# feixue94/pram

Hardware: AMD Instinct MI355X
Metric: query images/sec (640x480, 2048 kpts, 7Scenes nc113) (higher is better)
Workload: dtype f32 results via split-fp16 MFMA (f16 x3 products, f32 accumulate); 1 GPU; 7Scenes full hot path: SFD2 extract+sample -> SegNetViT nc113 (15 layers) -> GML match + 20 Sinkhorn iters, 2048 query kpts vs a 2048-kpt reference set; stages=erm; precision=x3, batches_in_flight_per_gpu=3, hipgraph_replay=False, attention_chunk_keys=4096, frame=640x480, keypoints=2048, parallelism=query-sharded x1, one all-gather of result records, matches_last_step=14291, matches_correct_last_step=14288, gather_order_verified=True

## Files before the change

### include/pram_hip.h

```cpp
#ifndef PRAM_HIP_H
#define PRAM_HIP_H

#include <stddef.h>
#include <stdint.h>

#ifdef __cplusplus
extern "C" {
#endif

#define PRAM_OK 0
#define PRAM_E_ARG (-1)
#define PRAM_E_LAUNCH (-2)
#define PRAM_E_UNSUPPORTED (-3)

int pram_hip_version(void);
const char* pram_last_error(void);

#define PRAM_STATUS_X3_RANGE 1u
int pram_set_status_word(unsigned int* device_word);
float pram_x3_set_act_scale(float scale);
int pram_read_status_word(unsigned int* host_out, int reset, void* stream);


#define PRAM_LIN_ROTARY 1
// ... 182 lines not shown
int pram_score_map_f32(const float* logits, float* score, int batch, int hc, int wc, void* stream);

size_t pram_simple_nms_workspace_bytes(int batch, int h, int w);
int pram_simple_nms_f32(const float* score, float* nms, int batch, int h, int w, int radius,
                        void* workspace, void* stream);

size_t pram_select_keypoints_workspace_bytes(int batch, int h, int w, int max_keypoints);

int pram_select_keypoints_f32(const float* nms, int batch, int h, int w, float conf_th,
                              int min_keypoints, int border, int max_keypoints, int fallback_ref,
                              float* kpts, float* scores, int* counts, void* workspace, void* stream);

int pram_sample_nhwc_f32(const float* fmap, int batch, int fh, int fw, int c, const float* kpts,
                         const int* lens, int n_max, int s, int l2norm, float* out, void* stream);

int pram_l2norm_rows_f32(float* x, int rows, int cols, void* stream);

int pram_score_lookup_f32(const float* score_map, long long map_stride, int h, int w, const float* kpts,
                          const int* lens, int batch, int n_max, float* out, void* stream);


int pram_resize_bilinear_f32(const float* in, float* out, int planes, int h, int w, int oh, int ow,
                             void* stream);

int pram_seg_epilogue_f32(const float* logits, const int* lens, int batch, int n_max, int n_class,
                          float bg_threshold, float* seg_scores, int* seg_ids, int* non_bg_mask,
                          int* n_non_bg, void* stream);

int pram_row_sort_desc_f32(const float* x, int ld, int rows, int cols, float* vals, long long* idx,
                           void* stream);
// ... 92 lines not shown
```

### pram_amd/_lib.py

```python
from __future__ import annotations

import ctypes as C
from pathlib import Path

import os as _os
_LIB_PATH = Path(_os.environ["PRAM_HIP_LIB"]) if _os.environ.get("PRAM_HIP_LIB") else Path(__file__).resolve().parent / "csrc" / "libpram_hip.so"
_lib = None

P = C.c_void_p
I = C.c_int
F = C.c_float
LL = C.c_longlong
SZ = C.c_size_t

_SIGS = {
    "pram_hip_version": (I, []),
    "pram_last_error": (C.c_char_p, []),
    "pram_set_status_word": (I, [P]),
    "pram_read_status_word": (I, [P, I, P]),
    "pram_x3_set_act_scale": (F, [F]),
    "pram_linear_f32": (I, [P, I, I, P, I, I, P, P, P, I, P, I, I, I, F, I, P, P, I, P]),
    "pram_linear_f16_f32": (I, [P, I, I, P, I, I, P, P, P, I, P, I, I, I, F, I, P, P, I, P]),
    "pram_linear_f16_ragged_f32": (I, [P, I, I, P, I, I, P, P, P, I, P, I, I, I, F, I, P, P, I, P, I, P]),
    "pram_linear_f16_h16": (I, [P, I, I, P, I, I, P, P, P, I, P, I, P, I, I, I, F, I, P, P, I, P]),
# ... 42 lines not shown
    "pram_adagml_scores4_f32": (I, [P, P, P, LL, P]),
    "pram_adagml_prune_ld_f32": (I, [P, I, F, I, P, P, P, P, P, P, P, P, P, P, P, P, P, I, I, I, P]),
    "pram_adagml_scatter_f32": (I, [P, P, P, P, P, I, I, I, P, P, P]),
    "pram_conv2d_nhwc_f32": (I, [P, I, I, I, I, P, P, P, P, P, P, I, I, I, I, P]),
    "pram_conv2d_nhwc_f16_f32": (I, [P, I, I, I, I, P, P, P, P, P, P, I, I, I, I, P]),
    "pram_conv3x3_grouped_nhwc_f32": (I, [P, I, I, I, I, P, P, P, P, I, I, P]),
    "pram_image_to_nhwc4_f32": (I, [P, P, I, I, I, P]),
    "pram_nhwc_to_nchw_f32": (I, [P, P, I, I, I, I, P]),
    "pram_score_map_f32": (I, [P, P, I, I, I, P]),
    "pram_simple_nms_workspace_bytes": (SZ, [I, I, I]),
    "pram_simple_nms_f32": (I, [P, P, I, I, I, I, P, P]),
    "pram_select_keypoints_workspace_bytes": (SZ, [I, I, I, I]),
    "pram_select_keypoints_f32": (I, [P, I, I, I, F, I, I, I, I, P, P, P, P, P]),
    "pram_sample_nhwc_f32": (I, [P, I, I, I, I, P, P, I, I, I, P, P]),
    "pram_l2norm_rows_f32": (I, [P, I, I, P]),
    "pram_resize_bilinear_f32": (I, [P, P, I, I, I, I, I, P]),
    "pram_seg_epilogue_f32": (I, [P, P, I, I, I, F, P, P, P, P, P]),
    "pram_row_sort_desc_f32": (I, [P, I, I, I, P, P, P]),
    "pram_row_top2_f32": (I, [P, I, LL, P, P, I, I, I, I, P, P, P, P]),
    "pram_proj_dist_top2_f32": (I, [P, I, P, P, I, I, F, P, P, P, P]),
    "pram_proj_dist_top2_f64uv": (I, [P, I, P, P, I, I, I, C.c_double, P, P, P, P]),
    "pram_project_points_f64": (I, [P, P, P, I, C.c_double, C.c_double, P, P, P, P, P, P]),
    "pram_seg_vote": (I, [P, P, I, I, I, P, P, P, P, P, P, P]),
    "pram_pack_record_f32": (I, [P, P, P, P, P, I, I, I, P, P]),
    "pram_fill_u32": (I, [P, C.c_uint, SZ, P]),
    "pram_stage_frames_u8": (I, [P, P, P, I, I, I, P]),
    "pram_score_lookup_f32": (I, [P, LL, I, I, P, P, I, I, P, P]),
    "pram_cand_mask_ranks": (I, [P, P, I, I, I, P]),
    "pram_cand_plan": (I, [P, P, P, P, P, I, I, I, I, P, P, P, I, I, P, P, P, P, I, I, C.c_double, I, P, P]),
    "pram_cand_gather": (I, [P, P, P, P, P, P, I, P, P, P, P, I, F, F, F, P, P, P, P, P, P, I, I, P]),
# ... 44 lines not shown
```

### pram_amd/csrc/conv.hip

```cpp
#include <stdlib.h>
#include "gemm_core.h"
#include "gemm_core_f16.h"
#include "gemm_core_x3.h"
#include "gemm_core_x3w.h"
#include "launch.h"

namespace {

struct ConvArgs {
    const float* in; const float* w; const float* bias; const float* scale; const float* shift;
    const float* residual; float* out;
    int batch, h, wd, cin, cout, ks, stride, relu;
    int ho, wo, m, k;
    int tiles_m, tiles_n;
    unsigned int* status;
    _Float16* out_hi; _Float16* out_lo;
    float act_scale = gemmx3::ACT_SCALE;
};

template <int MI, int WN>
__device__ __forceinline__ void conv_epilogue(const ConvArgs& p, f32x16 (&acc)[MI][2], int row0, int col0, int BM, int BN) {
    using gemm::acc_row;
    const int tid = threadIdx.x;
    const int nlast = p.cout - 1;
    const int lane = tid & 63, wave = tid >> 6;
    const int wm = wave / WN, wn = wave % WN;
    const int r = lane & 31, h = lane >> 5;
    const int mlast = p.m - 1;
    const int rbase = row0 + wm * 32 * MI;
    const bool full = (row0 + BM <= p.m) && (col0 + BN <= p.cout);
#pragma unroll
    for (int ni = 0; ni < 2; ++ni) {
        const int col = col0 + wn * 64 + ni * 32 + r;
// ... 254 lines not shown
        const bool in = (unsigned)iy < (unsigned)p.h && (unsigned)ix < (unsigned)p.wd;
        const unsigned off = in ? (unsigned)(roff[pp] + tap) : 0u;
        return *reinterpret_cast<const float4*>(base[pp] + off);
    };
    auto oka = [&](int pp, int kt) -> bool {
        const int iy = iy0[pp] + cky, ix = ix0[pp] + ckx;
        return ok[pp] && (unsigned)iy < (unsigned)p.h && (unsigned)ix < (unsigned)p.wd;
    };
    auto lb = [&](int pp, int kt) -> uint4 { return *reinterpret_cast<const uint4*>(brow16[pp] + koff); };
    auto okb = [&](int pp, int kt) -> bool { return (col0 + brow + 32 * pp) < p.cout; };
    f32x16 acc[MI][2];
    mainloop<MI, WN>(smem, adv, la, oka, lb, okb, p.k / BK, acc);
    conv_epilogue<MI, WN>(p, acc, row0, col0, BM, BN);
}

template <int MI, int WN, bool L2N = false>
__global__ __launch_bounds__(gemmx3::NT, 2) void conv_x3_kernel(ConvArgs p, const _Float16* __restrict__ wh,
                                                                 const _Float16* __restrict__ wl, float inv) {
    using namespace gemmx3;
    using C = Cfg<MI, WN>;
    constexpr int BM = C::BM, BN = C::BN;
    __shared__ Smem<MI, WN> smem;
    const int nblk = p.tiles_m * p.tiles_n;
    const int id = xcd_remap(blockIdx.x, nblk);
    const int tn = id % p.tiles_n, tm = id / p.tiles_n;
    const int tid = threadIdx.x;
    const int arow = tid >> 3, akq = tid & 7, brow = tid >> 2, bsl = tid & 3;
    const int row0 = tm * BM, col0 = tn * BN;
    const int pad = p.ks >> 1;
    int iy0[C::PA], ix0[C::PA], roff[C::PA];
    const float* base[C::PA];
    bool ok[C::PA];
#pragma unroll
    for (int pp = 0; pp < C::PA; ++pp) {
        const int row = row0 + arow + 32 * pp;
        ok[pp] = row < p.m;
        const int rr = ok[pp] ? row : 0;
        const int ox = rr % p.wo;
        const int t = rr / p.wo;
        const int oy = t % p.ho;
        const int b = t / p.ho;
        iy0[pp] = oy * p.stride - pad;
        ix0[pp] = ox * p.stride - pad;
// ... 25 lines not shown
    auto okb = [&](int pp, int kt) -> bool { return (col0 + brow + 64 * pp) < p.cout; };
    f32x16 acc[MI][2];
    float amax = 0.f;
    mainloop<MI, WN>(smem, adv, la, oka, lb, okb, p.k / BK, p.act_scale, acc, amax);
    x3_range_flag(p.status, amax);
#pragma unroll
    for (int mi = 0; mi < MI; ++mi)
#pragma unroll
        for (int ni = 0; ni < 2; ++ni)
#pragma unroll
            for (int e = 0; e < 16; ++e) acc[mi][ni][e] *= inv;
    if constexpr (L2N) conv_epilogue_l2norm<MI, WN>(p, acc, row0, col0, BM, reinterpret_cast<float*>(&smem));
    else conv_epilogue<MI, WN>(p, acc, row0, col0, BM, BN);
}

template <int MI, int WM, int WN, bool PLANES = false>
__global__ __launch_bounds__(64 * WM * WN, 2) void conv_x3w_kernel(ConvArgs p, const _Float16* __restrict__ wh,
                                                                    const _Float16* __restrict__ wl, float inv) {
    using namespace gemmx3w;
    using C = Cfg<MI, WM, WN>;
    constexpr int BM = C::BM, BN = C::BN;
    extern __shared__ __attribute__((aligned(16))) unsigned char smem_raw[];
    Smem<MI, WM, WN>& smem = *reinterpret_cast<Smem<MI, WM, WN>*>(smem_raw);
    const int nblk = p.tiles_m * p.tiles_n;
    const int id = xcd_remap(blockIdx.x, nblk);
    const int tn = id % p.tiles_n, tm = id / p.tiles_n;
    const int tid = threadIdx.x;
    const int arow = tid >> 3, akq = tid & 7, qrow = tid >> 2, qsl = tid & 3;
    const int row0 = tm * BM, col0 = tn * BN;
    const int pad = p.ks >> 1;
    int iy0[C::PA], ix0[C::PA], roff[C::PA];
    const float* base[C::PA];
    bool ok[C::PA];
#pragma unroll
    for (int pp = 0; pp < C::PA; ++pp) {
        const int row = row0 + arow + C::RA * pp;
        ok[pp] = row < p.m;
        const int rr = ok[pp] ? row : 0;
        const int ox = rr % p.wo;
        const int t = rr / p.wo;
        const int oy = t % p.ho;
        const int b = t / p.ho;
        iy0[pp] = oy * p.stride - pad;
        ix0[pp] = ox * p.stride - pad;
        base[pp] = p.in + (size_t)b * p.h * p.wd * p.cin;
        roff[pp] = (iy0[pp] * p.wd + ix0[pp]) * p.cin + akq * 4;
    }
    const int nlast = p.cout - 1;
    int cky = 0, ckx = 0, cci = 0, koff = 0, tap = 0;
    auto adv = [&](int kt) {
        if (kt == 0) { cky = ckx = cci = koff = tap = 0; return; }
        if (++ckx == p.ks) { ckx = 0; if (++cky == p.ks) { cky = 0; cci += BK; } }
        koff = (cky * p.ks + ckx) * p.cin + cci;
        tap = (cky * p.wd + ckx) * p.cin + cci;
    };
    size_t boff[C::QB];
#pragma unroll
// ... 467 lines not shown
    const char* who = "pram_conv2d_nhwc_x3_l2norm_f32";
    ConvArgs p{};
    p.in = in; p.bias = bias; p.scale = scale; p.shift = shift; p.residual = residual; p.out = out;
    p.batch = batch; p.h = h; p.wd = w; p.cin = cin; p.cout = cout; p.ks = ks; p.stride = stride; p.relu = relu;
    if (int e = conv_args(who, p, CONV_X3, in && wgt_hi && wgt_lo && out, w_scale)) return e;
    PRAM_REQUIRE(cout > 0 && cout <= 128, "%s: cout=%d must be at most 128", who, cout);
    if (batch == 0) return PRAM_OK;
    const float inv = arm_split(p, w_scale);
    p.tiles_m = cdiv(p.m, gemmx3::Cfg<2, 2>::BM);
    p.tiles_n = 1;
    hipLaunchKernelGGL((conv_x3_kernel<2, 2, true>), dim3(p.tiles_m), dim3(gemmx3::NT), 0, (hipStream_t)stream, p, (const _Float16*)wgt_hi,
                       (const _Float16*)wgt_lo, inv);
    return pram_launch_status(who);
}

extern "C" int pram_conv2d_nhwc_x3_planes(const float* in, int batch, int h, int w, int cin, const void* wgt_hi, const void* wgt_lo,
                                          float w_scale, const float* bias, const float* scale, const float* shift,
                                          const float* residual, void* out_hi, void* out_lo, int cout, int ks, int stride, int relu,
                                          void* stream) {
    const char* who = "pram_conv2d_nhwc_x3_planes";
    ConvArgs p{};
    p.in = in; p.bias = bias; p.scale = scale; p.shift = shift; p.residual = residual;
    p.batch = batch; p.h = h; p.wd = w; p.cin = cin; p.cout = cout; p.ks = ks; p.stride = stride; p.relu = relu;
    if (int e = conv_args(who, p, CONV_X3, in && wgt_hi && wgt_lo && out_hi && out_lo, w_scale)) return e;
    PRAM_REQUIRE(cout > 0 && cout % 2 == 0, "%s: cout=%d must be even", who, cout);
    if (batch == 0) return PRAM_OK;
    const float inv = arm_split(p, w_scale);
    p.out_hi = (_Float16*)out_hi;
    p.out_lo = (_Float16*)out_lo;
    using CW = gemmx3w::Cfg<4, 2, 4>;
// ... 226 lines not shown
```

### pram_amd/csrc/sfd2_post.hip

```cpp
#include "common.h"
#include <math.h>

namespace {

__global__ __launch_bounds__(256) void score_map_kernel(const float* __restrict__ logits, float* __restrict__ score,
                                                        int hc, int wc, int ncell) {
    const int lane = threadIdx.x & 63;
    const int cell = blockIdx.x * 4 + (threadIdx.x >> 6);
    if (cell >= ncell) return;
    const float* src = logits + (size_t)cell * 65;
    const float x = src[lane];
    const float xd = src[64];
    const float mx = fmaxf(wave_max(x), xd);
    const float e = expf(x - mx);
    const float sum = wave_sum(e) + expf(xd - mx);
    const int cx = cell % wc;
    const int t = cell / wc;
    const int cy = t % hc;
    const int b = t / hc;
    const int W = wc * 8;
    score[((size_t)b * hc * 8 + cy * 8 + (lane >> 3)) * W + cx * 8 + (lane & 7)] = e / sum;
}

constexpr int NMS_T = 32;
// ... 314 lines not shown
            }
            if (BIG) __threadfence_block();
            __syncthreads();
        }
    }
    for (int i = tid; i < kmax; i += SEL_T) {
        const unsigned long long kk = keys[i];
        const unsigned idx = 0xFFFFFFFFu - (unsigned)(kk & 0xFFFFFFFFull);
        ko[2 * i] = (float)(idx % w);
        ko[2 * i + 1] = (float)(idx / w);
        so[i] = __uint_as_float((unsigned)(kk >> 32));
    }
    if (tid == 0) counts[b] = kmax;
}

__global__ __launch_bounds__(256) void sample_kernel(const float* __restrict__ fmap, int fh, int fw, int c,
                                                     const float* __restrict__ kpts, const int* __restrict__ lens,
                                                     int n_max, float s, int l2norm, float* __restrict__ out) {
    const int b = blockIdx.y;
    const int lane = threadIdx.x & 63;
    const int n = blockIdx.x * 4 + (threadIdx.x >> 6);
    const int len = lens ? lens[b] : n_max;
    if (n >= len) return;
    const float kx = kpts[((size_t)b * n_max + n) * 2], ky = kpts[((size_t)b * n_max + n) * 2 + 1];
    float gx = kx, gy = ky;
    if (s > 0.f) {
        const float half = s * 0.5f;
        const float dx = (float)fw * s - half - 0.5f, dy = (float)fh * s - half - 0.5f;
        gx = (kx - half) + 0.5f;
        gy = (ky - half) + 0.5f;
        gx = gx / dx;
        gy = gy / dy;
        gx = gx * 2.f - 1.f;
        gy = gy * 2.f - 1.f;
    }
    const float ix = ((gx + 1.f) / 2.f) * (float)(fw - 1);
    const float iy = ((gy + 1.f) / 2.f) * (float)(fh - 1);
    const float fx0 = floorf(ix), fy0 = floorf(iy);
    const int x0 = (int)fx0, y0 = (int)fy0, x1 = x0 + 1, y1 = y0 + 1;
    const float wnw = ((fx0 + 1.f) - ix) * ((fy0 + 1.f) - iy);
    const float wne = (ix - fx0) * ((fy0 + 1.f) - iy);
    const float wsw = ((fx0 + 1.f) - ix) * (iy - fy0);
    const float wse = (ix - fx0) * (iy - fy0);
    const bool vx0 = (unsigned)x0 < (unsigned)fw, vx1 = (unsigned)x1 < (unsigned)fw;
    const bool vy0 = (unsigned)y0 < (unsigned)fh, vy1 = (unsigned)y1 < (unsigned)fh;
    const float* base = fmap + (size_t)b * fh * fw * c;
    float* dst = out + ((size_t)b * n_max + n) * c;
    auto gather = [&](int c4) -> float4 {
        float4 a = make_float4(0.f, 0.f, 0.f, 0.f);
        if (c4 * 4 < c) {
            auto tap = [&](bool ok, int yy, int xx, float wgt) {
                if (ok) {
                    const float4 v = *reinterpret_cast<const float4*>(base + ((size_t)yy * fw + xx) * c + c4 * 4);
                    a.x += v.x * wgt; a.y += v.y * wgt; a.z += v.z * wgt; a.w += v.w * wgt;
                }
            };
            tap(vx0 && vy0, y0, x0, wnw);
            tap(vx1 && vy0, y0, x1, wne);
            tap(vx0 && vy1, y1, x0, wsw);
            tap(vx1 && vy1, y1, x1, wse);
        }
        return a;
    };
    float4 a0 = gather(lane), a1 = gather(lane + 64);
    if (l2norm) {
        const float sq = ((a0.x * a0.x + a0.y * a0.y) + (a0.z * a0.z + a0.w * a0.w)) +
                         ((a1.x * a1.x + a1.y * a1.y) + (a1.z * a1.z + a1.w * a1.w));
        const float d = fmaxf(sqrtf(wave_sum(sq)), 1e-12f);
        a0.x /= d; a0.y /= d; a0.z /= d; a0.w /= d;
        a1.x /= d; a1.y /= d; a1.z /= d; a1.w /= d;
    }
    if (lane * 4 < c) *reinterpret_cast<float4*>(dst + lane * 4) = a0;
    if ((lane + 64) * 4 < c) *reinterpret_cast<float4*>(dst + (lane + 64) * 4) = a1;
}

__global__ __launch_bounds__(256) void l2norm_rows_kernel(float* __restrict__ x, int rows, int cols) {
    const int lane = threadIdx.x & 63;
    const int row = blockIdx.x * 4 + (threadIdx.x >> 6);
    if (row >= rows) return;
    float* p = x + (size_t)row * cols;
    float sq = 0.f;
    for (int c = lane * 4; c < cols; c += 256) {
        const float4 v = *reinterpret_cast<const float4*>(p + c);
        sq += (v.x * v.x + v.y * v.y) + (v.z * v.z + v.w * v.w);
    }
    const float d = fmaxf(sqrtf(wave_sum(sq)), 1e-12f);
    for (int c = lane * 4; c < cols; c += 256) {
        float4 v = *reinterpret_cast<const float4*>(p + c);
// ... 93 lines not shown
    hipLaunchKernelGGL(sel_count_kernel, dim3(SEL_SLABS, batch), dim3(256), 0, st, nms, h, w, slab_px, conf_th, border, ws);
    hipLaunchKernelGGL(sel_compact_kernel, dim3(SEL_SLABS, batch), dim3(256), 0, st, nms, h, w, slab_px, conf_th, min_keypoints, border,
                       fallback_ref, ws);
    if (ws.keys) hipLaunchKernelGGL(sel_select_kernel<true>, dim3(batch), dim3(SEL_T), 0, st, nms, h, w, conf_th, min_keypoints, border,
                                    max_keypoints, fallback_ref, ws, kpts, scores, counts);
    else hipLaunchKernelGGL(sel_select_kernel<false>, dim3(batch), dim3(SEL_T), 0, st, nms, h, w, conf_th, min_keypoints, border,
                            max_keypoints, fallback_ref, ws, kpts, scores, counts);
    return pram_launch_status("pram_select_keypoints_f32");
}

extern "C" int pram_sample_nhwc_f32(const float* fmap, int batch, int fh, int fw, int c, const float* kpts, const int* lens,
                                    int n_max, int s, int l2norm, float* out, void* stream) {
    PRAM_REQUIRE(fmap && kpts && out, "pram_sample_nhwc_f32: null pointer");
    PRAM_REQUIRE(c % 4 == 0 && c <= 512, "pram_sample_nhwc_f32: c=%d must be a multiple of 4 and <= 512", c);
    if (batch == 0 || n_max == 0) return PRAM_OK;
    hipLaunchKernelGGL(sample_kernel, dim3(cdiv(n_max, 4), batch), dim3(256), 0, (hipStream_t)stream, fmap, fh, fw, c, kpts,
                       lens, n_max, (float)s, l2norm, out);
    return pram_launch_status("pram_sample_nhwc_f32");
}

extern "C" int pram_l2norm_rows_f32(float* x, int rows, int cols, void* stream) {
    PRAM_REQUIRE(x && cols % 4 == 0, "pram_l2norm_rows_f32: cols must be a multiple of 4");
    if (rows == 0) return PRAM_OK;
    hipLaunchKernelGGL(l2norm_rows_kernel, dim3(cdiv(rows, 4)), dim3(256), 0, (hipStream_t)stream, x, rows, cols);
    return pram_launch_status("pram_l2norm_rows_f32");
}

extern "C" int pram_score_lookup_f32(const float* score_map, long long map_stride, int h, int w, const float* kpts,
                                     const int* lens, int batch, int n_max, float* out, void* stream) {
    PRAM_REQUIRE(score_map && kpts && out, "pram_score_lookup_f32: null pointer");
    if (batch == 0 || n_max == 0) return PRAM_OK;
    hipLaunchKernelGGL(score_lookup_kernel, dim3(cdiv(n_max, 256), batch), dim3(256), 0, (hipStream_t)stream, score_map,
                       map_stride, h, w, kpts, lens, n_max, out);
// ... 3 lines not shown
```

### pram_amd/nets/sfd2.py

```python
from __future__ import annotations

from typing import Dict, List, Optional

import torch
import torch.nn as nn

from .. import ops
from . import _blocks as blk

RGB_mean = [0.485, 0.456, 0.406]
RGB_std = [0.229, 0.224, 0.225]


def norm_RGB(img: torch.Tensor) -> torch.Tensor:
    mean = img.new_tensor(RGB_mean).view(-1, 1, 1)
    std = img.new_tensor(RGB_std).view(-1, 1, 1)
    return (img - mean) / std


def _conv_bn(cin, cout, stride=1):
    return nn.Sequential(nn.Conv2d(cin, cout, 3, stride, 1), nn.BatchNorm2d(cout), nn.ReLU(inplace=True))


class _Res(nn.Module):
# ... 86 lines not shown
            if ops.GROUPED_X3 and ops.gemm_prec() == "x3" and o4.shape[-1] % 64 == 0 and o4.numel() < (1 << 29):
                yh, yl = ops.conv2d_nhwc_planes(o4, P[p + ".w1"], None, P[p + ".s1"], P[p + ".t1"], ks=1, relu=True)
                y = ops.conv3x3_grouped_planes(yh, yl, P[p + ".w2"], P[p + ".s2"], P[p + ".t2"], groups=o4.shape[-1] // 8, relu=True)
            else:
                y = ops.conv2d_nhwc(o4, P[p + ".w1"], None, P[p + ".s1"], P[p + ".t1"], ks=1, relu=True)
                y = ops.conv3x3_grouped_nhwc(y, P[p + ".w2"], P[p + ".s2"], P[p + ".t2"], groups=32, relu=True)
            o4 = ops.conv2d_nhwc(y, P[p + ".w3"], None, P[p + ".s3"], P[p + ".t3"], residual=o4, ks=1, relu=True)
        return P, o1b, o2b, o3b, o4

    def _score_head(self, P, o4):
        pa = ops.conv2d_nhwc(o4, P["convPa.w0"], P["convPa.b0"], P["convPa.s0"], P["convPa.t0"], ks=3, stride=2, relu=True)
        pa = ops.conv2d_nhwc(pa, P["convPa.w3"], P["convPa.b3"], ks=3)
        logits = ops.conv2d_nhwc(pa, P["convPb.w"], P["convPb.b"], ks=1)
        return logits, ops.score_map(logits)

    def _desc_head(self, P, o4):
        da = ops.conv2d_nhwc(o4, P["convDa.w0"], P["convDa.b0"], P["convDa.s0"], P["convDa.t0"], ks=3, relu=True)
        da = ops.conv2d_nhwc(da, P["convDa.w3"], P["convDa.b3"], ks=3)
        return ops.conv2d_nhwc(da, P["convDb.w"], P["convDb.b"], ks=1, l2norm=True)

    @staticmethod
    def _nchw_view(x_nhwc: torch.Tensor) -> torch.Tensor:
        return x_nhwc.permute(0, 3, 1, 2)

    @torch.no_grad()
    @blk.with_model_precision
    def det(self, x):
        P, _, _, _, o4 = self._backbone(x)
        _, score = self._score_head(P, o4)
        return score, self._nchw_view(self._desc_head(P, o4))

    @torch.no_grad()
    @blk.with_model_precision
    def forward(self, batch):
        P, _, _, _, o4 = self._backbone(batch['image'])
        logits, score = self._score_head(P, o4)
        desc = self._nchw_view(self._desc_head(P, o4))
        lg = self._nchw_view(logits)
        return {'dense_features': desc, 'scores': score, 'logits': lg, 'semi_map': torch.softmax(lg, 1)[:, :-1]}

    def extract_patches(self, batch):
        return self.forward(batch)

    @torch.no_grad()
    @blk.with_model_precision
    def extract_batched(self, image: torch.Tensor, config: dict, per_image_fallback: bool = True):
        cfg = {**self.default_config, **config}
        b, _, ih, iw = image.shape
        P, o1b, o2b, o3b, o4 = self._backbone(image)
        _, score = self._score_head(P, o4)
        if score.shape[1] != ih or score.shape[2] != iw:
            score = ops.resize_bilinear(score, ih, iw)
        nms = ops.simple_nms(score, 4)
        if cfg['max_keypoints'] < 0:
            kpts, scores, counts = ops.select_keypoints(nms, cfg['conf_th'], cfg['min_keypoints'], cfg['remove_borders'],
                                                        ih * iw, -1 if per_image_fallback else 0)
            k_eff = max(int(counts.max().item()), 1)
            kpts, scores = kpts[:, :k_eff].contiguous(), scores[:, :k_eff].contiguous()
        else:
            kpts, scores, counts = ops.select_keypoints(nms, cfg['conf_th'], cfg['min_keypoints'], cfg['remove_borders'],
                                                        cfg['max_keypoints'], -1 if per_image_fallback else 0)
        desc_map = self._desc_head(P, o4)
        descs = ops.sample_nhwc(desc_map, kpts, counts, 4, True)
        return dict(score_map=score, desc_map=desc_map, mid_features=o4, global_nhwc=[o1b, o2b, o3b, o4],
                    keypoints=kpts, scores=scores, descriptors=descs, counts=counts)

    @torch.no_grad()
    def extract_local_global(self, data, config={'conf_th': 0.005, 'remove_borders': 4, 'min_keypoints': 128,
                                                 'max_keypoints': 4096}):
        r = self.extract_batched(data['image'], config, per_image_fallback=False)
        counts: List[int] = r['counts'].tolist()
        return {
            'score_map': r['score_map'],
            'desc_map': self._nchw_view(r['desc_map']),
            'mid_features': self._nchw_view(r['mid_features']),
            'global_descriptors': [self._nchw_view(t) for t in r['global_nhwc']],
            'keypoints': [r['keypoints'][i, :c] for i, c in enumerate(counts)],
            'scores': [r['scores'][i, :c] for i, c in enumerate(counts)],
# ... 125 lines not shown
```

### pram_amd/ops.py

```python
from __future__ import annotations

from typing import Optional, Tuple

import torch

from . import _lib

_INT64 = torch.int64


def _st() -> int:
    return torch.cuda.current_stream().cuda_stream


def _p(t: Optional[torch.Tensor]) -> Optional[int]:
    return None if t is None else t.data_ptr()


def _chk(t: torch.Tensor, name: str, dtype=torch.float32):
    if not t.is_cuda:
        raise _lib.PramHipError(f"{name}: expected a CUDA tensor (pram_amd has no CPU path)")
    if t.dtype != dtype:
        raise _lib.PramHipError(f"{name}: expected {dtype}, got {t.dtype}")

# ... 980 lines not shown
    return kpts, scores, counts


def sample_nhwc(fmap: torch.Tensor, kpts: torch.Tensor, lens: Optional[torch.Tensor], s: int, l2norm: bool) -> torch.Tensor:
    L = _lib.load()
    assert fmap.is_contiguous()
    kpts = kpts.contiguous()
    B, fh, fw, Cc = fmap.shape
    N = kpts.shape[1]
    out = _filled((B, N, Cc), fmap.device)
    _lib.check(L.pram_sample_nhwc_f32(_p(fmap), B, fh, fw, Cc, _p(kpts), _p(lens), N, int(s), int(l2norm), _p(out), _st()),
               "pram_sample_nhwc_f32")
    return out


def l2norm_rows_(x: torch.Tensor) -> torch.Tensor:
    L = _lib.load()
    assert x.is_contiguous()
    cols = x.shape[-1]
    _lib.check(L.pram_l2norm_rows_f32(_p(x), x.numel() // cols, cols, _st()), "pram_l2norm_rows_f32")
    return x


def score_lookup(score_map_: torch.Tensor, kpts: torch.Tensor, lens: Optional[torch.Tensor]) -> torch.Tensor:
    L = _lib.load()
    score_map_ = score_map_.contiguous()
    kpts = kpts.contiguous()
    B, H, W = score_map_.shape
    Bk, N = kpts.shape[0], kpts.shape[1]
    out = _filled((Bk, N), kpts.device)
# ... 363 lines not shown
```

### pram_amd/pipeline.py

```python
from __future__ import annotations

from typing import Dict, Optional

import torch

from . import ops


import threading as _threading

_BRANCH = {}
_BRANCH_LOCK = _threading.Lock()


def _branch_stream(device, main: Optional[torch.cuda.Stream] = None) -> torch.cuda.Stream:
    import time
    dev = torch.device(device)
    main = main or torch.cuda.current_stream(dev)
    key = (dev.index if dev.index is not None else torch.cuda.current_device(), main.cuda_stream)
    with _BRANCH_LOCK:
        if key in _BRANCH:
            return _BRANCH[key]
    if torch.cuda.is_current_stream_capturing():
        raise RuntimeError("pram_amd.pipeline: the side stream of a forked step has to be measured before a stream capture — call "
# ... 14 lines not shown
    for _ in range(8):
        c = torch.cuda.Stream(device=dev)
        spin([main, c])
        t = min(spin([main, c]) for _ in range(2))
        if t < best_t:
            best, best_t = c, t
        if t < 1.5 * one:
            break
    with _BRANCH_LOCK:
        return _BRANCH.setdefault(key, best)


class QueryPipeline:

    def __init__(self, sfd2, segnet, matcher, max_keypoints: int = 2048, min_keypoints: int = 128, bg_threshold: float = 0.95,
                 overlap_below: int = 8, guard: str = "fallback", match_keypoints: int = 0):
        self.sfd2, self.segnet, self.matcher = sfd2, segnet, matcher
        self.bg_threshold = bg_threshold
        self.cfg = {'min_keypoints': min_keypoints, 'max_keypoints': max_keypoints}
        self.overlap_below = overlap_below
        self.guard = guard
        self.match_keypoints = int(match_keypoints)
        self._side, self._side_main = None, None

    def warm_up(self, device, main: Optional[torch.cuda.Stream] = None) -> None:
        dev = torch.device(device)
        main = main or torch.cuda.current_stream(dev)
        self._side, self._side_main = _branch_stream(dev, main), main.cuda_stream

    def _match(self, ex, ref, W, H):
        kpts, scores, counts, desc = ex['keypoints'], ex['scores'], ex['counts'], ex['descriptors']
        km = self.match_keypoints
        if 0 < km < kpts.shape[1]:
            kpts, scores, desc = kpts[:, :km].contiguous(), scores[:, :km].contiguous(), desc[:, :km].contiguous()
            counts = torch.clamp(counts, max=km)
        data = {
            'descriptors0': desc, 'keypoints0': kpts, 'scores0': scores, 'lens0': counts,
            'image_shape0': (1, 3, W, H),
            'descriptors1': ref['descriptors'], 'keypoints1': ref['keypoints'], 'scores1': ref['scores'],
            'image_shape1': (1, 3, W, H),
        }
        if 'lens' in ref:
            data['lens1'] = ref['lens']
        return self.matcher.produce_matches(data) if hasattr(self.matcher, 'produce_matches') else self.matcher(data)

    @torch.no_grad()
    def run(self, images: torch.Tensor, ref: Optional[Dict[str, torch.Tensor]] = None, stages: str = "erm",
            guard: Optional[str] = None) -> Dict[str, torch.Tensor]:
        with ops.guard_scope(guard or self.guard):
            return ops.guarded_call(lambda: self._run(images, ref, stages), images.device)

    def _extract(self, images):
        return self.sfd2.extract_batched(images, self.cfg, per_image_fallback=True)

    def _recognise(self, ex, images, out):
        kpts, counts = ex['keypoints'], ex['counts']
        _, seg = self.sfd2.sample_batched(ex['score_map'], ex['mid_features'], kpts, counts, norm_desc=False)
        pred = self.segnet({'seg_descriptors': seg, 'keypoints': kpts, 'image': images, 'lens': counts})['prediction']
        out['prediction'] = pred
        ids, non_bg, n_non_bg, _ = ops.seg_epilogue(pred, counts, self.bg_threshold)
        out['landmark'], out['non_bg'], out['n_non_bg'] = ids, non_bg, n_non_bg

    def _forks(self, batch: int, ref, stages: str) -> bool:
        return 'm' in stages and ref is not None and 'r' in stages and batch < self.overlap_below

    def _run(self, images, ref, stages):
        B, _, H, W = images.shape
        ex = self._extract(images)
# ... 170 lines not shown
```

Measured before the change: 623.8 queries/s.

## Compute SFD2 descriptor head only at pixels touched by keypoint bilinear taps

Adds a row-list kernel that marks, in an LDS bitmap, every feature-map pixel one of the four bilinear taps of a keypoint reads. It then compacts those pixels into a per-image row list with a pixel-to-row map. The second 3x3 conv and the 1x1 conv with l2norm of the descriptor head then run only over those rows, through a gather variant of the x3 conv kernel and a tile-skipping variant of the 1x1 kernel. A row-indirected sampler reads the final descriptors. The pipeline now defaults to this sparse path, which drops dense work on pixels no keypoint samples, at the cost of an extra launch, indirect gathers, and a dense-map output that is no longer produced.

```diff
diff --git a/include/pram_hip.h b/include/pram_hip.h
--- a/include/pram_hip.h
+++ b/include/pram_hip.h
@@ -220,6 +220,20 @@
 int pram_sample_nhwc_f32(const float* fmap, int batch, int fh, int fw, int c, const float* kpts,
                          const int* lens, int n_max, int s, int l2norm, float* out, void* stream);
 
+
+int pram_sfd2_row_list(const float* kpts, const int* lens, int batch, int n_max, int fh, int fw, int s, int* rows,
+                       int* n_rows, int* pix2row, int rlen, void* stream);
+
+int pram_conv3x3_rows_x3_f32(const float* in, int batch, int h, int w, int cin, const void* wgt_hi, const void* wgt_lo,
+                             float w_scale, const float* bias, const int* rows, const int* n_rows, int rlen, float* out,
+                             int cout, int relu, void* stream);
+
+int pram_conv1x1_rows_x3_l2norm_f32(const float* in, int batch, int rlen, int cin, const void* wgt_hi, const void* wgt_lo,
+                                    float w_scale, const float* bias, const int* n_rows, float* out, int cout, void* stream);
+
+int pram_sample_rows_f32(const float* rowmap, const int* pix2row, int batch, int rlen, int fh, int fw, int c, const float* kpts,
+                         const int* lens, int n_max, int s, int l2norm, float* out, void* stream);
+
 int pram_l2norm_rows_f32(float* x, int rows, int cols, void* stream);
 
 int pram_score_lookup_f32(const float* score_map, long long map_stride, int h, int w, const float* kpts,
diff --git a/pram_amd/_lib.py b/pram_amd/_lib.py
--- a/pram_amd/_lib.py
+++ b/pram_amd/_lib.py
@@ -80,6 +80,10 @@
     "pram_select_keypoints_f32": (I, [P, I, I, I, F, I, I, I, I, P, P, P, P, P]),
     "pram_sample_nhwc_f32": (I, [P, I, I, I, I, P, P, I, I, I, P, P]),
     "pram_l2norm_rows_f32": (I, [P, I, I, P]),
+    "pram_sfd2_row_list": (I, [P, P, I, I, I, I, I, P, P, P, I, P]),
+    "pram_conv3x3_rows_x3_f32": (I, [P, I, I, I, I, P, P, F, P, P, P, I, P, I, I, P]),
+    "pram_conv1x1_rows_x3_l2norm_f32": (I, [P, I, I, I, P, P, F, P, P, P, I, P]),
+    "pram_sample_rows_f32": (I, [P, P, I, I, I, I, I, P, P, I, I, I, P, P]),
     "pram_resize_bilinear_f32": (I, [P, P, I, I, I, I, I, P]),
     "pram_seg_epilogue_f32": (I, [P, P, I, I, I, F, P, P, P, P, P]),
     "pram_row_sort_desc_f32": (I, [P, I, I, I, P, P, P]),
diff --git a/pram_amd/csrc/conv.hip b/pram_amd/csrc/conv.hip
--- a/pram_amd/csrc/conv.hip
+++ b/pram_amd/csrc/conv.hip
@@ -16,7 +16,10 @@
     unsigned int* status;
     _Float16* out_hi; _Float16* out_lo;
     float act_scale = gemmx3::ACT_SCALE;
+    const int* rows = nullptr; const int* n_rows = nullptr; int rlen = 0;
 };
+
+constexpr int ROWS_BM = 256;
 
 template <int MI, int WN>
 __device__ __forceinline__ void conv_epilogue(const ConvArgs& p, f32x16 (&acc)[MI][2], int row0, int col0, int BM, int BN) {
@@ -301,7 +304,7 @@
     conv_epilogue<MI, WN>(p, acc, row0, col0, BM, BN);
 }
 
-template <int MI, int WN, bool L2N = false>
+template <int MI, int WN, bool L2N = false, bool ROWS = false>
 __global__ __launch_bounds__(gemmx3::NT, 2) void conv_x3_kernel(ConvArgs p, const _Float16* __restrict__ wh,
                                                                  const _Float16* __restrict__ wl, float inv) {
     using namespace gemmx3;
@@ -314,6 +317,11 @@
     const int tid = threadIdx.x;
     const int arow = tid >> 3, akq = tid & 7, brow = tid >> 2, bsl = tid & 3;
     const int row0 = tm * BM, col0 = tn * BN;
+    if constexpr (ROWS) {
+        static_assert(ROWS_BM % BM == 0, "a tile must lie inside one producer tile");
+        const int fb = row0 / p.rlen;
+        if ((row0 - fb * p.rlen) / ROWS_BM * ROWS_BM >= p.n_rows[fb]) return;
+    }
     const int pad = p.ks >> 1;
     int iy0[C::PA], ix0[C::PA], roff[C::PA];
     const float* base[C::PA];
@@ -369,7 +377,7 @@
     else conv_epilogue<MI, WN>(p, acc, row0, col0, BM, BN);
 }
 
-template <int MI, int WM, int WN, bool PLANES = false>
+template <int MI, int WM, int WN, bool PLANES = false, bool GATHER = false>
 __global__ __launch_bounds__(64 * WM * WN, 2) void conv_x3w_kernel(ConvArgs p, const _Float16* __restrict__ wh,
                                                                     const _Float16* __restrict__ wl, float inv) {
     using namespace gemmx3w;
@@ -384,6 +392,14 @@
     const int arow = tid >> 3, akq = tid & 7, qrow = tid >> 2, qsl = tid & 3;
     const int row0 = tm * BM, col0 = tn * BN;
     const int pad = p.ks >> 1;
+    int seg = 0, seg_row0 = 0, live = 0;
+    if constexpr (GATHER) {
+        static_assert(BM == ROWS_BM, "the row-list chain's skip rule is written for this tile");
+        seg = row0 / p.rlen;
+        seg_row0 = row0 - seg * p.rlen;
+        live = p.n_rows[seg];
+        if (seg_row0 >= live) return;
+    }
     int iy0[C::PA], ix0[C::PA], roff[C::PA];
     const float* base[C::PA];
     bool ok[C::PA];
@@ -392,10 +408,16 @@
         const int row = row0 + arow + C::RA * pp;
         ok[pp] = row < p.m;
         const int rr = ok[pp] ? row : 0;
-        const int ox = rr % p.wo;
+        int ox = rr % p.wo;
         const int t = rr / p.wo;
-        const int oy = t % p.ho;
-        const int b = t / p.ho;
+        int oy = t % p.ho;
+        int b = t / p.ho;
+        if constexpr (GATHER) {
+            const int px = p.rows[(size_t)seg * p.rlen + min(seg_row0 + arow + C::RA * pp, live - 1)];
+            oy = px / p.wo;
+            ox = px - oy * p.wo;
+            b = seg;
+        }
         iy0[pp] = oy * p.stride - pad;
         ix0[pp] = ox * p.stride - pad;
         base[pp] = p.in + (size_t)b * p.h * p.wd * p.cin;
@@ -893,6 +915,49 @@
     return pram_launch_status(who);
 }
 
+extern "C" int pram_conv3x3_rows_x3_f32(const float* in, int batch, int h, int w, int cin, const void* wgt_hi, const void* wgt_lo,
+                                        float w_scale, const float* bias, const int* rows, const int* n_rows, int rlen, float* out,
+                                        int cout, int relu, void* stream) {
+    const char* who = "pram_conv3x3_rows_x3_f32";
+    ConvArgs p{};
+    p.in = in; p.bias = bias; p.out = out;
+    p.batch = batch; p.h = h; p.wd = w; p.cin = cin; p.cout = cout; p.ks = 3; p.stride = 1; p.relu = relu;
+    if (int e = conv_args(who, p, CONV_X3, in && wgt_hi && wgt_lo && out && rows && n_rows, w_scale)) return e;
+    PRAM_REQUIRE(cout > 0 && rlen > 0 && rlen % ROWS_BM == 0 && (long long)batch * rlen < (1ll << 31),
+                 "%s: rlen=%d must be a positive multiple of %d (batch * rlen < 2^31), cout=%d positive", who, rlen, ROWS_BM, cout);
+    if (batch == 0) return PRAM_OK;
+    const float inv = arm_split(p, w_scale);
+    p.rows = rows; p.n_rows = n_rows; p.rlen = rlen;
+    p.m = batch * rlen;
+    using CW = gemmx3w::Cfg<4, 2, 4>;
+    static_assert(CW::BM == ROWS_BM, "ROWS_BM is this tile's height");
+    const size_t shm = sizeof(gemmx3w::Smem<4, 2, 4>);
+    opt_in_lds<conv_x3w_kernel<4, 2, 4, false, true>>(shm);
+    hipLaunchKernelGGL((conv_x3w_kernel<4, 2, 4, false, true>), dim3(set_tiles<CW>(p, cout)), dim3(CW::NT), shm, (hipStream_t)stream, p,
+                       (const _Float16*)wgt_hi, (const _Float16*)wgt_lo, inv);
+    return pram_launch_status(who);
+}
+
+extern "C" int pram_conv1x1_rows_x3_l2norm_f32(const float* in, int batch, int rlen, int cin, const void* wgt_hi, const void* wgt_lo,
+                                               float w_scale, const float* bias, const int* n_rows, float* out, int cout, void* stream) {
+    const char* who = "pram_conv1x1_rows_x3_l2norm_f32";
+    ConvArgs p{};
+    p.in = in; p.bias = bias; p.out = out;
+    PRAM_REQUIRE(batch >= 0 && rlen > 0 && rlen % ROWS_BM == 0 && (long long)batch * rlen < (1ll << 31),
+                 "%s: rlen=%d must be a positive multiple of %d (batch * rlen < 2^31)", who, rlen, ROWS_BM);
+    p.batch = 1; p.h = 1; p.wd = batch * rlen; p.cin = cin; p.cout = cout; p.ks = 1; p.stride = 1; p.relu = 0;
+    if (int e = conv_args(who, p, CONV_X3, in && wgt_hi && wgt_lo && out && n_rows, w_scale)) return e;
+    PRAM_REQUIRE(cout > 0 && cout <= 128, "%s: cout=%d must be at most 128", who, cout);
+    if (batch == 0) return PRAM_OK;
+    const float inv = arm_split(p, w_scale);
+    p.n_rows = n_rows; p.rlen = rlen;
+    p.tiles_m = cdiv(p.m, gemmx3::Cfg<2, 2>::BM);
+    p.tiles_n = 1;
+    hipLaunchKernelGGL((conv_x3_kernel<2, 2, true, true>), dim3(p.tiles_m), dim3(gemmx3::NT), 0, (hipStream_t)stream, p,
+                       (const _Float16*)wgt_hi, (const _Float16*)wgt_lo, inv);
+    return pram_launch_status(who);
+}
+
 extern "C" int pram_conv2d_nhwc_x3_planes(const float* in, int batch, int h, int w, int cin, const void* wgt_hi, const void* wgt_lo,
                                           float w_scale, const float* bias, const float* scale, const float* shift,
                                           const float* residual, void* out_hi, void* out_lo, int cout, int ks, int stride, int relu,
diff --git a/pram_amd/csrc/sfd2_post.hip b/pram_amd/csrc/sfd2_post.hip
--- a/pram_amd/csrc/sfd2_post.hip
+++ b/pram_amd/csrc/sfd2_post.hip
@@ -352,15 +352,13 @@
     if (tid == 0) counts[b] = kmax;
 }
 
-__global__ __launch_bounds__(256) void sample_kernel(const float* __restrict__ fmap, int fh, int fw, int c,
-                                                     const float* __restrict__ kpts, const int* __restrict__ lens,
-                                                     int n_max, float s, int l2norm, float* __restrict__ out) {
-    const int b = blockIdx.y;
-    const int lane = threadIdx.x & 63;
-    const int n = blockIdx.x * 4 + (threadIdx.x >> 6);
-    const int len = lens ? lens[b] : n_max;
-    if (n >= len) return;
-    const float kx = kpts[((size_t)b * n_max + n) * 2], ky = kpts[((size_t)b * n_max + n) * 2 + 1];
+struct Corners {
+    int x0, y0;
+    float wnw, wne, wsw, wse;
+    bool vx0, vx1, vy0, vy1;
+};
+
+__device__ __forceinline__ Corners sample_corners(float kx, float ky, int fh, int fw, float s) {
     float gx = kx, gy = ky;
     if (s > 0.f) {
         const float half = s * 0.5f;
@@ -375,28 +373,54 @@
     const float ix = ((gx + 1.f) / 2.f) * (float)(fw - 1);
     const float iy = ((gy + 1.f) / 2.f) * (float)(fh - 1);
     const float fx0 = floorf(ix), fy0 = floorf(iy);
-    const int x0 = (int)fx0, y0 = (int)fy0, x1 = x0 + 1, y1 = y0 + 1;
-    const float wnw = ((fx0 + 1.f) - ix) * ((fy0 + 1.f) - iy);
-    const float wne = (ix - fx0) * ((fy0 + 1.f) - iy);
-    const float wsw = ((fx0 + 1.f) - ix) * (iy - fy0);
-    const float wse = (ix - fx0) * (iy - fy0);
-    const bool vx0 = (unsigned)x0 < (unsigned)fw, vx1 = (unsigned)x1 < (unsigned)fw;
-    const bool vy0 = (unsigned)y0 < (unsigned)fh, vy1 = (unsigned)y1 < (unsigned)fh;
-    const float* base = fmap + (size_t)b * fh * fw * c;
+    Corners c;
+    c.x0 = (int)fx0;
+    c.y0 = (int)fy0;
+    c.wnw = ((fx0 + 1.f) - ix) * ((fy0 + 1.f) - iy);
+    c.wne = (ix - fx0) * ((fy0 + 1.f) - iy);
+    c.wsw = ((fx0 + 1.f) - ix) * (iy - fy0);
+    c.wse = (ix - fx0) * (iy - fy0);
+    c.vx0 = (unsigned)c.x0 < (unsigned)fw;
+    c.vx1 = (unsigned)(c.x0 + 1) < (unsigned)fw;
+    c.vy0 = (unsigned)c.y0 < (unsigned)fh;
+    c.vy1 = (unsigned)(c.y0 + 1) < (unsigned)fh;
+    return c;
+}
+
+__device__ __forceinline__ int live_keypoints(const int* __restrict__ lens, int b, int n_max) {
+    return min(lens ? lens[b] : n_max, n_max);
+}
+
+template <bool ROWS>
+__global__ __launch_bounds__(256) void sample_kernel(const float* __restrict__ fmap, int fh, int fw, int c,
+                                                     const float* __restrict__ kpts, const int* __restrict__ lens,
+                                                     int n_max, float s, int l2norm, float* __restrict__ out,
+                                                     const int* __restrict__ pix2row, int rlen) {
+    const int b = blockIdx.y;
+    const int lane = threadIdx.x & 63;
+    const int n = blockIdx.x * 4 + (threadIdx.x >> 6);
+    const int len = live_keypoints(lens, b, n_max);
+    if (n >= len) return;
+    const float kx = kpts[((size_t)b * n_max + n) * 2], ky = kpts[((size_t)b * n_max + n) * 2 + 1];
+    const Corners k = sample_corners(kx, ky, fh, fw, s);
+    const int x0 = k.x0, y0 = k.y0, x1 = x0 + 1, y1 = y0 + 1;
+    const float* base = fmap + (size_t)b * (ROWS ? rlen : fh * fw) * c;
+    const int* p2r = ROWS ? pix2row + (size_t)b * fh * fw : nullptr;
     float* dst = out + ((size_t)b * n_max + n) * c;
     auto gather = [&](int c4) -> float4 {
         float4 a = make_float4(0.f, 0.f, 0.f, 0.f);
         if (c4 * 4 < c) {
             auto tap = [&](bool ok, int yy, int xx, float wgt) {
                 if (ok) {
-                    const float4 v = *reinterpret_cast<const float4*>(base + ((size_t)yy * fw + xx) * c + c4 * 4);
+                    const int px = yy * fw + xx;
+                    const float4 v = *reinterpret_cast<const float4*>(base + (size_t)(ROWS ? p2r[px] : px) * c + c4 * 4);
                     a.x += v.x * wgt; a.y += v.y * wgt; a.z += v.z * wgt; a.w += v.w * wgt;
                 }
             };
-            tap(vx0 && vy0, y0, x0, wnw);
-            tap(vx1 && vy0, y0, x1, wne);
-            tap(vx0 && vy1, y1, x0, wsw);
-            tap(vx1 && vy1, y1, x1, wse);
+            tap(k.vx0 && k.vy0, y0, x0, k.wnw);
+            tap(k.vx1 && k.vy0, y0, x1, k.wne);
+            tap(k.vx0 && k.vy1, y1, x0, k.wsw);
+            tap(k.vx1 && k.vy1, y1, x1, k.wse);
         }
         return a;
     };
@@ -410,6 +434,68 @@
     }
     if (lane * 4 < c) *reinterpret_cast<float4*>(dst + lane * 4) = a0;
     if ((lane + 64) * 4 < c) *reinterpret_cast<float4*>(dst + (lane + 64) * 4) = a1;
+}
+
+constexpr int RL_T = 1024;
+
+__global__ __launch_bounds__(RL_T) void row_list_kernel(const float* __restrict__ kpts, const int* __restrict__ lens, int n_max,
+                                                        int fh, int fw, float s, int* __restrict__ rows, int* __restrict__ n_rows,
+                                                        int* __restrict__ pix2row, int rlen) {
+    extern __shared__ unsigned int rl_bits[];
+    const int b = blockIdx.x, tid = threadIdx.x, lane = tid & 63, wave = tid >> 6;
+    const int npix = fh * fw, nwords = (npix + 31) >> 5;
+    unsigned int* wtot = rl_bits + nwords;
+    for (int i = tid; i < nwords; i += RL_T) rl_bits[i] = 0u;
+    __syncthreads();
+    const int len = live_keypoints(lens, b, n_max);
+    for (int n = tid; n < len; n += RL_T) {
+        const Corners k = sample_corners(kpts[((size_t)b * n_max + n) * 2], kpts[((size_t)b * n_max + n) * 2 + 1], fh, fw, s);
+        auto mark = [&](bool ok, int yy, int xx) {
+            if (ok) {
+                const int px = yy * fw + xx;
+                atomicOr(&rl_bits[px >> 5], 1u << (px & 31));
+            }
+        };
+        mark(k.vx0 && k.vy0, k.y0, k.x0);
+        mark(k.vx1 && k.vy0, k.y0, k.x0 + 1);
+        mark(k.vx0 && k.vy1, k.y0 + 1, k.x0);
+        mark(k.vx1 && k.vy1, k.y0 + 1, k.x0 + 1);
+    }
+    __syncthreads();
+    const int wpt = (nwords + RL_T - 1) / RL_T;
+    const int w0 = min(tid * wpt, nwords), w1 = min(w0 + wpt, nwords);
+    int cnt = 0;
+    for (int w = w0; w < w1; ++w) cnt += __popc(rl_bits[w]);
+    int inc = cnt;
+#pragma unroll
+    for (int o = 1; o < 64; o <<= 1) {
+        const int v = __shfl_up(inc, o, 64);
+        if (lane >= o) inc += v;
+    }
+    if (lane == 63) wtot[wave] = (unsigned int)inc;
+    __syncthreads();
+    int before = 0, total = 0;
+#pragma unroll
+    for (int w = 0; w < RL_T / 64; ++w) {
+        const int t = (int)wtot[w];
+        if (w < wave) before += t;
+        total += t;
+    }
+    int pos = before + inc - cnt;
+    int* rb = rows + (size_t)b * rlen;
+    int* pb = pix2row + (size_t)b * npix;
+    for (int w = w0; w < w1; ++w) {
+        unsigned int m = rl_bits[w];
+        while (m) {
+            const int px = (w << 5) + __ffs((int)m) - 1;
+            m &= m - 1;
+            rb[pos] = px;
+            pb[px] = pos;
+            ++pos;
+        }
+    }
+    for (int i = total + tid; i < rlen; i += RL_T) rb[i] = -1;
+    if (tid == 0) n_rows[b] = total;
 }
 
 __global__ __launch_bounds__(256) void l2norm_rows_kernel(float* __restrict__ x, int rows, int cols) {
@@ -533,9 +619,33 @@
     PRAM_REQUIRE(fmap && kpts && out, "pram_sample_nhwc_f32: null pointer");
     PRAM_REQUIRE(c % 4 == 0 && c <= 512, "pram_sample_nhwc_f32: c=%d must be a multiple of 4 and <= 512", c);
     if (batch == 0 || n_max == 0) return PRAM_OK;
-    hipLaunchKernelGGL(sample_kernel, dim3(cdiv(n_max, 4), batch), dim3(256), 0, (hipStream_t)stream, fmap, fh, fw, c, kpts,
-                       lens, n_max, (float)s, l2norm, out);
+    hipLaunchKernelGGL(sample_kernel<false>, dim3(cdiv(n_max, 4), batch), dim3(256), 0, (hipStream_t)stream, fmap, fh, fw, c, kpts,
+                       lens, n_max, (float)s, l2norm, out, (const int*)nullptr, 0);
     return pram_launch_status("pram_sample_nhwc_f32");
+}
+
+extern "C" int pram_sfd2_row_list(const float* kpts, const int* lens, int batch, int n_max, int fh, int fw, int s, int* rows,
+                                  int* n_rows, int* pix2row, int rlen, void* stream) {
+    PRAM_REQUIRE(kpts && rows && n_rows && pix2row, "pram_sfd2_row_list: null pointer");
+    PRAM_REQUIRE(fh > 0 && fw > 0 && (long long)fh * fw <= (1 << 18), "pram_sfd2_row_list: a map of %d x %d pixels does not fit the LDS bitmap (2^18)", fh, fw);
+    PRAM_REQUIRE(n_max >= 0 && rlen > 0 && (long long)rlen >= (4ll * n_max < (long long)fh * fw ? 4ll * n_max : (long long)fh * fw),
+                 "pram_sfd2_row_list: rlen=%d is less than min(4 * n_max, fh * fw)", rlen);
+    if (batch == 0) return PRAM_OK;
+    const size_t shm = ((size_t)(fh * fw + 31) / 32 + RL_T / 64) * sizeof(unsigned int);
+    hipLaunchKernelGGL(row_list_kernel, dim3(batch), dim3(RL_T), shm, (hipStream_t)stream, kpts, lens, n_max, fh, fw, (float)s, rows,
+                       n_rows, pix2row, rlen);
+    return pram_launch_status("pram_sfd2_row_list");
+}
+
+extern "C" int pram_sample_rows_f32(const float* rowmap, const int* pix2row, int batch, int rlen, int fh, int fw, int c, const float* kpts,
+                                    const int* lens, int n_max, int s, int l2norm, float* out, void* stream) {
+    PRAM_REQUIRE(rowmap && pix2row && kpts && out, "pram_sample_rows_f32: null pointer");
+    PRAM_REQUIRE(c % 4 == 0 && c <= 512, "pram_sample_rows_f32: c=%d must be a multiple of 4 and <= 512", c);
+    PRAM_REQUIRE(rlen > 0 && (long long)fh * fw < (1ll << 31), "pram_sample_rows_f32: bad sizes rlen=%d fh=%d fw=%d", rlen, fh, fw);
+    if (batch == 0 || n_max == 0) return PRAM_OK;
+    hipLaunchKernelGGL(sample_kernel<true>, dim3(cdiv(n_max, 4), batch), dim3(256), 0, (hipStream_t)stream, rowmap, fh, fw, c, kpts,
+                       lens, n_max, (float)s, l2norm, out, pix2row, rlen);
+    return pram_launch_status("pram_sample_rows_f32");
 }
 
 extern "C" int pram_l2norm_rows_f32(float* x, int rows, int cols, void* stream) {
diff --git a/pram_amd/nets/sfd2.py b/pram_amd/nets/sfd2.py
--- a/pram_amd/nets/sfd2.py
+++ b/pram_amd/nets/sfd2.py
@@ -124,9 +124,11 @@
         logits = ops.conv2d_nhwc(pa, P["convPb.w"], P["convPb.b"], ks=1)
         return logits, ops.score_map(logits)
 
+    def _desc_stem(self, P, o4):
+        return ops.conv2d_nhwc(o4, P["convDa.w0"], P["convDa.b0"], P["convDa.s0"], P["convDa.t0"], ks=3, relu=True)
+
     def _desc_head(self, P, o4):
-        da = ops.conv2d_nhwc(o4, P["convDa.w0"], P["convDa.b0"], P["convDa.s0"], P["convDa.t0"], ks=3, relu=True)
-        da = ops.conv2d_nhwc(da, P["convDa.w3"], P["convDa.b3"], ks=3)
+        da = ops.conv2d_nhwc(self._desc_stem(P, o4), P["convDa.w3"], P["convDa.b3"], ks=3)
         return ops.conv2d_nhwc(da, P["convDb.w"], P["convDb.b"], ks=1, l2norm=True)
 
     @staticmethod
@@ -154,7 +156,7 @@
 
     @torch.no_grad()
     @blk.with_model_precision
-    def extract_batched(self, image: torch.Tensor, config: dict, per_image_fallback: bool = True):
+    def extract_batched(self, image: torch.Tensor, config: dict, per_image_fallback: bool = True, dense_desc: bool = True):
         cfg = {**self.default_config, **config}
         b, _, ih, iw = image.shape
         P, o1b, o2b, o3b, o4 = self._backbone(image)
@@ -170,8 +172,13 @@
         else:
             kpts, scores, counts = ops.select_keypoints(nms, cfg['conf_th'], cfg['min_keypoints'], cfg['remove_borders'],
                                                         cfg['max_keypoints'], -1 if per_image_fallback else 0)
-        desc_map = self._desc_head(P, o4)
-        descs = ops.sample_nhwc(desc_map, kpts, counts, 4, True)
+        if not dense_desc and cfg['max_keypoints'] >= 0 and ops.gemm_prec() == "x3":
+            desc_map = None
+            descs = ops.sampled_descriptors(self._desc_stem(P, o4), P["convDa.w3"], P["convDa.b3"], P["convDb.w"], P["convDb.b"],
+                                            kpts, counts, 4)
+        else:
+            desc_map = self._desc_head(P, o4)
+            descs = ops.sample_nhwc(desc_map, kpts, counts, 4, True)
         return dict(score_map=score, desc_map=desc_map, mid_features=o4, global_nhwc=[o1b, o2b, o3b, o4],
                     keypoints=kpts, scores=scores, descriptors=descs, counts=counts)
 
diff --git a/pram_amd/ops.py b/pram_amd/ops.py
--- a/pram_amd/ops.py
+++ b/pram_amd/ops.py
@@ -1018,6 +1018,53 @@
     return out
 
 
+SPARSE_DESC_MAX_FRACTION = 0.9
+SPARSE_ROWS_TILE = 256
+
+
+def sparse_desc_rows(n_max: int, fh: int, fw: int) -> int:
+    r = -(-min(4 * n_max, fh * fw) // SPARSE_ROWS_TILE) * SPARSE_ROWS_TILE
+    return r if 0 < r < SPARSE_DESC_MAX_FRACTION * fh * fw and fh * fw <= (1 << 18) else 0
+
+
+def sparse_descriptors(x: torch.Tensor, w3: torch.Tensor, b3, w1: torch.Tensor, b1, kpts: torch.Tensor, lens: Optional[torch.Tensor],
+                       s: int, rlen: int, want_parts: bool = False):
+    L = _lib.load()
+    _chk(x, "x")
+    assert x.is_contiguous() and w3.is_contiguous() and w1.is_contiguous()
+    kpts = kpts.contiguous()
+    B, fh, fw, Cin = x.shape
+    N = kpts.shape[1]
+    Cm, Cout = w3.shape[0], w1.shape[0]
+    dev = x.device
+    rows = torch.empty(B, rlen, device=dev, dtype=torch.int32)
+    n_rows = torch.empty(B, device=dev, dtype=torch.int32)
+    pix2row = torch.empty(B, fh * fw, device=dev, dtype=torch.int32)
+    _lib.check(L.pram_sfd2_row_list(_p(kpts), _p(lens), B, N, fh, fw, int(s), _p(rows), _p(n_rows), _p(pix2row), rlen, _st()),
+               "pram_sfd2_row_list")
+    mid = torch.empty(B * rlen, Cm, device=dev, dtype=torch.float32)
+    wh, wl, ws = split_weight(w3)
+    _lib.check(L.pram_conv3x3_rows_x3_f32(_p(x), B, fh, fw, Cin, _p(wh), _p(wl), ws, _p(b3), _p(rows), _p(n_rows), rlen, _p(mid), Cm, 0,
+                                          _st()), "pram_conv3x3_rows_x3_f32")
+    dmat = torch.empty(B * rlen, Cout, device=dev, dtype=torch.float32)
+    wh, wl, ws = split_weight(w1)
+    _lib.check(L.pram_conv1x1_rows_x3_l2norm_f32(_p(mid), B, rlen, Cm, _p(wh), _p(wl), ws, _p(b1), _p(n_rows), _p(dmat), Cout, _st()),
+               "pram_conv1x1_rows_x3_l2norm_f32")
+    out = _filled((B, N, Cout), dev)
+    _lib.check(L.pram_sample_rows_f32(_p(dmat), _p(pix2row), B, rlen, fh, fw, Cout, _p(kpts), _p(lens), N, int(s), 1, _p(out), _st()),
+               "pram_sample_rows_f32")
+    return (out, rows, n_rows, pix2row) if want_parts else out
+
+
+def sampled_descriptors(x: torch.Tensor, w3: torch.Tensor, b3, w1: torch.Tensor, b1, kpts: torch.Tensor, lens: Optional[torch.Tensor],
+                        s: int) -> torch.Tensor:
+    rlen = sparse_desc_rows(kpts.shape[1], x.shape[1], x.shape[2]) if FUSED_L2NORM else 0
+    if rlen:
+        return sparse_descriptors(x, w3, b3, w1, b1, kpts, lens, s, rlen)
+    dm = conv2d_nhwc(conv2d_nhwc(x, w3, b3, ks=3, precision="x3"), w1, b1, ks=1, precision="x3", l2norm=True)
+    return sample_nhwc(dm, kpts, lens, s, True)
+
+
 def l2norm_rows_(x: torch.Tensor) -> torch.Tensor:
     L = _lib.load()
     assert x.is_contiguous()
diff --git a/pram_amd/pipeline.py b/pram_amd/pipeline.py
--- a/pram_amd/pipeline.py
+++ b/pram_amd/pipeline.py
@@ -52,7 +52,7 @@
 class QueryPipeline:
 
     def __init__(self, sfd2, segnet, matcher, max_keypoints: int = 2048, min_keypoints: int = 128, bg_threshold: float = 0.95,
-                 overlap_below: int = 8, guard: str = "fallback", match_keypoints: int = 0):
+                 overlap_below: int = 8, guard: str = "fallback", match_keypoints: int = 0, dense_desc: bool = False):
         self.sfd2, self.segnet, self.matcher = sfd2, segnet, matcher
         self.bg_threshold = bg_threshold
         self.cfg = {'min_keypoints': min_keypoints, 'max_keypoints': max_keypoints}
@@ -60,6 +60,7 @@
         self.guard = guard
         self.match_keypoints = int(match_keypoints)
         self._side, self._side_main = None, None
+        self.dense_desc = bool(dense_desc)
 
     def warm_up(self, device, main: Optional[torch.cuda.Stream] = None) -> None:
         dev = torch.device(device)
@@ -89,7 +90,7 @@
             return ops.guarded_call(lambda: self._run(images, ref, stages), images.device)
 
     def _extract(self, images):
-        return self.sfd2.extract_batched(images, self.cfg, per_image_fallback=True)
+        return self.sfd2.extract_batched(images, self.cfg, per_image_fallback=True, dense_desc=self.dense_desc)
 
     def _recognise(self, ex, images, out):
         kpts, counts = ex['keypoints'], ex['counts']
```

After: 638.2 queries/s, median of 6. 2.3% higher.
